# ErikNatanael/knaster

Hardware: AMD Instinct MI355X
Metric: UGen-samples/sec (voices x block_size x UGens / s) (higher is better)
Workload: dtype f32

## Files before the change

knaster_amd/csrc/bank.hip:

```cpp
#include <hip/hip_runtime.h>

#include <algorithm>
#include <atomic>
#include <chrono>
#include <cmath>
#include <cstddef>
#include <cstdio>
#include <cstdlib>
#include <cstring>
#include <functional>
#include <memory>
#include <mutex>
#include <new>
#include <stdexcept>
#include <string>
#include <thread>
#include <vector>

#include "../../include/knaster_hip.h"
#include "jit.hpp"
#include "kernel_form.hpp"
#include "kernel_registry.hpp"

using knh_dev::Event;
// ... 310 lines not shown
    return create_bank(desc, k >= 2 && k <= 64 ? static_cast<uint32_t>(k) : 0u, out_bank);
  });
}

int32_t knh_bank_create_sharded(const knh_bank_desc* desc, uint32_t host_threads, knh_bank** out_bank) {
  return guarded(nullptr, [&]() -> int32_t {
    return create_bank(desc, host_threads, out_bank);
  });
}

void knh_bank_destroy(knh_bank* bank) {
  try {
    if (bank && bank->pipe_stream) {
      (void)hipSetDevice(bank->device);
      (void)hipStreamSynchronize(bank->pipe_stream);
    }
    delete bank;
  } catch (...) {
  }
}

int32_t knh_bank_set_ctor_args(knh_bank* bank, uint32_t stage, uint32_t first_voice, uint32_t count, const double* args, uint32_t n_args) {
  return guarded(bank, [&]() -> int32_t {
    if (!bank) return KNH_ERR_INVALID_ARGUMENT;
    return bank->set_ctor(stage, first_voice, count, args, n_args);
  });
}
int32_t knh_bank_set_buffer(knh_bank* bank, uint32_t stage, const void* samples, size_t n_frames, double buffer_sample_rate) {
  return guarded(bank, [&]() -> int32_t {
    if (!bank) return KNH_ERR_INVALID_ARGUMENT;
// ... 226 lines not shown
int32_t knh_bank_process_blocks_device_add(knh_bank* bank, uint32_t n_blocks, uint64_t frame_clock, void* out_device, void* hip_stream) {
  return guarded(bank, [&]() -> int32_t {
    if (!bank) return KNH_ERR_INVALID_ARGUMENT;
    return bank->process(n_blocks, bank->block_size, 0, frame_clock, nullptr, out_device, nullptr, nullptr, hip_stream, false, true);
  });
}
int32_t knh_bank_process_blocks_begin(knh_bank* bank, uint32_t n_blocks, uint64_t frame_clock) {
  return guarded(bank, [&]() -> int32_t {
    if (!bank) return KNH_ERR_INVALID_ARGUMENT;
    if (!bank->initialised) return bank->fail(KNH_ERR_NOT_INITIALISED, "bank not initialised");
    if (bank->pipe_count == 2) return bank->fail(KNH_ERR_INVALID_ARGUMENT, "two launches are outstanding: fetch one with knh_bank_process_blocks_end first");
    if (n_blocks == 0 || n_blocks > 4096) return bank->fail(KNH_ERR_INVALID_ARGUMENT, "n_blocks must be in 1..4096");
    auto hip = [&](hipError_t e, const char* what) { return e == hipSuccess ? KNH_OK : bank->fail(KNH_ERR_DEVICE, std::string(what) + ": " + hipGetErrorString(e)); };
    int rc = hip(hipSetDevice(bank->device), "hipSetDevice");
    if (rc != KNH_OK) return rc;
    if (!bank->pipe_stream && (rc = hip(hipStreamCreateWithFlags(&bank->pipe_stream, hipStreamNonBlocking), "hipStreamCreate")) != KNH_OK) return rc;
    knh_bank::PipeSlot& p = bank->pipe[(bank->pipe_head + bank->pipe_count) % 2];
    const size_t bytes = static_cast<size_t>(n_blocks) * bank->desc.out_channels * bank->block_size * (bank->desc.sample_type == KNH_F64 ? 8 : 4);
    if (bytes > p.cap) {
      if (p.dev) (void)hipFree(p.dev);
      if (p.host) (void)hipHostFree(p.host);
      p.dev = p.host = nullptr;
      p.cap = 0;
      if ((rc = hip(hipMalloc(&p.dev, bytes), "hipMalloc")) != KNH_OK) return rc;
      if ((rc = hip(hipMemset(p.dev, 0, bytes), "hipMemset")) != KNH_OK) return rc;
      if ((rc = hip(hipHostMalloc(&p.host, bytes), "hipHostMalloc")) != KNH_OK) return rc;
      p.cap = bytes;
    }
    if (!p.done && (rc = hip(hipEventCreateWithFlags(&p.done, hipEventDisableTiming), "hipEventCreate")) != KNH_OK) return rc;
    p.bytes = bytes;
    rc = bank->process(n_blocks, bank->block_size, 0, frame_clock, nullptr, p.dev, nullptr, nullptr, bank->pipe_stream, false);
// ... 132 lines not shown
```

knaster_amd/csrc/kernel_registry.hpp:

```cpp
#pragma once
#include <hip/hip_runtime.h>

#include "voice_chain.hpp"

namespace knh_dev {
enum { INTERP_VAL_MUL = 0, INTERP_VAL_ADD, INTERP_VAL_SUB, INTERP_VAL_DIV, INTERP_VAL_VSUB, INTERP_VAL_VDIV, INTERP_VAL_LAST = INTERP_VAL_VDIV,
       INTERP_MATH_MUL, INTERP_MATH_ADD, INTERP_MATH_SUB, INTERP_MATH_DIV, INTERP_SIN_WT,
       INTERP_MATH1_CEIL, INTERP_MATH1_SQRT, INTERP_MATH1_FLOOR, INTERP_MATH1_TRUNC, INTERP_MATH1_FRACT, INTERP_MATH1_EXP };
struct InterpOp { u32 kind; unsigned short a, b, o, pad; u32 slot; };
static_assert(sizeof(InterpOp) == 16, "one 16-byte LDS read per stage");
struct DevRec {
  u32 voice;
  unsigned short delay;
  unsigned short stage;
  unsigned char param;
  unsigned char kb;
  unsigned short block;
  u32 pad;
  u64 value;
};
static_assert(sizeof(DevRec) == 24, "one 24-byte record per call");
struct DevStage {
  unsigned short kind, dcpb, slot_base, param_base, flags, ar_param;
  short widx;
// ... 30 lines not shown
  u32 seg_max;
  void* delay_ring;
  u32 n_rings;
  u64 ring_base[16];
  u32 ring_stride[16];
};
}

namespace knh {
hipError_t launch_resolve_events(const knh_dev::EventResolveArgs& a, hipStream_t s);
hipError_t launch_restart_voices(const knh_dev::RestartArgs& a, unsigned count, hipStream_t s);

template <typename F>
using VoiceLaunchFn = hipError_t (*)(const knh_dev::VoiceKernelArgs<F>& args, unsigned n_wavefronts, hipStream_t stream);

struct KernelEntry {
  const char* signature;
  int n_slots;
  VoiceLaunchFn<float> f32[2];
  VoiceLaunchFn<double> f64[2];
};
struct PipeEntry {
  const char* signature;
  int n_groups;
  int form;
  int gpw;
  int long_tiles;
  VoiceLaunchFn<float> f32[2];
  VoiceLaunchFn<double> f64[2];
};
// ... 14 lines not shown
hipError_t launch_interp_f64(const knh_dev::VoiceKernelArgs<double>& a, const knh_dev::InterpOp* prog, unsigned n_ops, unsigned n_state_words,
                             unsigned n_sig, unsigned out_sig, double* rows, hipStream_t s);

const KernelEntry* find_kernel(const char* signature);
int kernel_count();
const KernelEntry* kernel_at(int i);

hipError_t launch_res_server_f32(const knh_dev::ResServerArgs<float>& a, hipStream_t s);
hipError_t launch_res_server_f64(const knh_dev::ResServerArgs<double>& a, hipStream_t s);
hipError_t launch_fold_f32(bool tree, const float* rows, unsigned n_rows, unsigned row_len, unsigned frame_begin,
                           unsigned frame_end, float* out, unsigned channels, unsigned out_stride, unsigned n_blocks, bool accumulate,
                           unsigned* zero_flags, hipStream_t s, const knh_dev::HostDone* host = nullptr);
hipError_t launch_fold_f64(bool tree, const double* rows, unsigned n_rows, unsigned row_len, unsigned frame_begin,
                           unsigned frame_end, double* out, unsigned channels, unsigned out_stride, unsigned n_blocks, bool accumulate,
                           unsigned* zero_flags, hipStream_t s, const knh_dev::HostDone* host = nullptr);

hipError_t launch_sum_shards_f32(const float* shards, unsigned n_shards, size_t shard_stride, size_t n, unsigned block_size,
                                 unsigned frame_begin, unsigned frame_end, float* out, bool accumulate, hipStream_t s);
hipError_t launch_sum_shards_f64(const double* shards, unsigned n_shards, size_t shard_stride, size_t n, unsigned block_size,
                                 unsigned frame_begin, unsigned frame_end, double* out, bool accumulate, hipStream_t s);

}
```

knaster_amd/csrc/kernels_fold.hip:

```cpp
#include <cstring>

#include "kernel_registry.hpp"
#include "voice_pipe.hpp"

namespace knh {
using namespace knh_dev;

template <typename F>
static hipError_t launch_fold(bool tree, const F* rows, unsigned n_rows, unsigned row_len, unsigned frame_begin, unsigned frame_end,
                              F* out, unsigned channels, unsigned out_stride, unsigned n_blocks, bool accumulate, unsigned* zero_flags,
                              const HostDone& host, hipStream_t s) {
  if (frame_end <= frame_begin || n_rows == 0 || n_blocks == 0) {
    if (host.words) return hipErrorInvalidValue;
    return zero_flags ? hipMemsetAsync(zero_flags, 0, 2 * sizeof(unsigned), s) : hipSuccess;
  }
  if (tree) {
    unsigned grid = (frame_end - frame_begin + 15u) / 16u;
    hipLaunchKernelGGL((fold_tree_kernel<F>), dim3(grid, n_blocks), dim3(256), 0, s, rows, n_rows, row_len, frame_begin, frame_end,
                       out, channels, out_stride, accumulate ? 1u : 0u, zero_flags, host);
  } else {
    unsigned grid = (frame_end - frame_begin + 63u) / 64u;
    hipLaunchKernelGGL((fold_rows_kernel<F>), dim3(grid, n_blocks), dim3(64), 0, s, rows, n_rows, row_len, frame_begin, frame_end,
                       out, channels, out_stride, accumulate ? 1u : 0u, zero_flags, host);
  }
  return hipGetLastError();
}
hipError_t launch_fold_f32(bool tree, const float* rows, unsigned n_rows, unsigned row_len, unsigned frame_begin,
                           unsigned frame_end, float* out, unsigned channels, unsigned out_stride, unsigned n_blocks, bool accumulate,
                           unsigned* zero_flags, hipStream_t s, const knh_dev::HostDone* host) {
  return launch_fold<float>(tree, rows, n_rows, row_len, frame_begin, frame_end, out, channels, out_stride, n_blocks, accumulate, zero_flags,
                            host ? *host : HostDone{nullptr, nullptr, nullptr, 0u}, s);
}
hipError_t launch_fold_f64(bool tree, const double* rows, unsigned n_rows, unsigned row_len, unsigned frame_begin,
                           unsigned frame_end, double* out, unsigned channels, unsigned out_stride, unsigned n_blocks, bool accumulate,
                           unsigned* zero_flags, hipStream_t s, const knh_dev::HostDone* host) {
  return launch_fold<double>(tree, rows, n_rows, row_len, frame_begin, frame_end, out, channels, out_stride, n_blocks, accumulate, zero_flags,
                             host ? *host : HostDone{nullptr, nullptr, nullptr, 0u}, s);
}


hipError_t launch_res_server_f32(const knh_dev::ResServerArgs<float>& a, hipStream_t s) {
  hipLaunchKernelGGL((res_fold_server<float>), dim3((a.n_rows + 31u) / 32u + 1u), dim3(256), 0, s, a);
  return hipGetLastError();
}
hipError_t launch_res_server_f64(const knh_dev::ResServerArgs<double>& a, hipStream_t s) {
  hipLaunchKernelGGL((res_fold_server<double>), dim3((a.n_rows + 31u) / 32u + 1u), dim3(256), 0, s, a);
  return hipGetLastError();
}

template <typename F>
__global__ void __launch_bounds__(256) sum_shards_kernel(const F* shards, unsigned n_shards, size_t shard_stride, size_t n,
                                                         unsigned block_size, unsigned frame_begin, unsigned frame_end, F* out,
                                                         unsigned accumulate) {
  const size_t i = (size_t)blockIdx.x * 256u + threadIdx.x;
// ... 26 lines not shown
```

knaster_amd/csrc/kernels_pipe.hip:

```cpp
#include <cstring>

#include "kernel_registry.hpp"
#include "voice_pipe.hpp"

namespace knh {
using namespace knh_dev;

template <typename F, bool FMA, int FORM, typename... Gs>
static hipError_t launch_pipe(const VoiceKernelArgs<F>& args, unsigned n_wavefronts, hipStream_t stream) {
  if (n_wavefronts == 0) return hipSuccess;
  constexpr int T = FORM != PIPE_MIXER ? PipeTile<F>::big : PipeTile<F>::value;
  hipLaunchKernelGGL((voice_pipe_kernel<F, FMA, T, FORM, 1, Gs...>), dim3(n_wavefronts), dim3(PipeWaves<T, FORM, Gs...>::value * 64), 0, stream, args);
  return hipGetLastError();
}
template <typename F, bool FMA, typename... Gs>
static hipError_t launch_pipe_pair(const VoiceKernelArgs<F>& args, unsigned n_wavefronts, hipStream_t stream) {
  if (n_wavefronts == 0) return hipSuccess;
  constexpr int T = PipeTile<F>::value;
  hipLaunchKernelGGL((voice_pipe_kernel<F, FMA, T, PIPE_INPLACE, 2, Gs...>), dim3((n_wavefronts + 1u) / 2u),
                     dim3(2 * PipeWaves<T, PIPE_INPLACE, Gs...>::value * 64), 0, stream, args);
  return hipGetLastError();
}
template <typename F, bool FMA, typename... Gs>
static hipError_t launch_pipe_wide_tile(const VoiceKernelArgs<F>& args, unsigned n_wavefronts, hipStream_t stream) {
  if (n_wavefronts == 0) return hipSuccess;
  constexpr int T = PipeTile<F>::big;
  hipLaunchKernelGGL((voice_pipe_kernel<F, FMA, T, PIPE_MIXER, 1, Gs...>), dim3(n_wavefronts), dim3(PipeWaves<T, PIPE_MIXER, Gs...>::value * 64), 0, stream, args);
  return hipGetLastError();
}
#define KNH_PIPE_FAN(sig, n, ...)                                                                                       \
  {sig, n, PIPE_MIXER, 1, 1, {launch_pipe_wide_tile<float, false, __VA_ARGS__>, launch_pipe_wide_tile<float, true, __VA_ARGS__>}, \
   {launch_pipe_wide_tile<double, false, __VA_ARGS__>, launch_pipe_wide_tile<double, true, __VA_ARGS__>}}
#define KNH_PIPE_AS(sig, n, form, ...)                                                               \
  {sig, n, form, 1, form != PIPE_MIXER ? 1 : 0, {launch_pipe<float, false, form, __VA_ARGS__>, launch_pipe<float, true, form, __VA_ARGS__>}, \
   {launch_pipe<double, false, form, __VA_ARGS__>, launch_pipe<double, true, form, __VA_ARGS__>}}
#define KNH_PIPE_PAIR_AS(sig, n, ...)                                                                \
  {sig, n, PIPE_INPLACE, 2, 0, {launch_pipe_pair<float, false, __VA_ARGS__>, launch_pipe_pair<float, true, __VA_ARGS__>}, \
   {launch_pipe_pair<double, false, __VA_ARGS__>, launch_pipe_pair<double, true, __VA_ARGS__>}},
#ifndef KNH_PIPE_PART
#error "KNH_PIPE_PART: 0, 1 or 2 (knaster_amd/build.py)"
#endif
#if KNH_PIPE_PART == 0
// ... 88 lines not shown
```

knaster_amd/csrc/kernels_single.hip:

```cpp
#include <cstring>

#include "kernel_registry.hpp"
#include "voice_pipe.hpp"

namespace knh {
using namespace knh_dev;

template <typename F, bool FMA, typename... S>
static hipError_t launch_voice(const VoiceKernelArgs<F>& args, unsigned n_wavefronts, hipStream_t stream) {
  if (n_wavefronts == 0) return hipSuccess;
  hipLaunchKernelGGL((voice_kernel<F, FMA, 1, S...>), dim3(n_wavefronts), dim3(64), 0, stream, args);
  return hipGetLastError();
}

#define KNH_CHAIN(sig, ...)                                                                  \
  {sig, Chain<float, false, 0, __VA_ARGS__>::kSlots,                                         \
   {launch_voice<float, false, __VA_ARGS__>, launch_voice<float, true, __VA_ARGS__>},        \
   {launch_voice<double, false, __VA_ARGS__>, launch_voice<double, true, __VA_ARGS__>}}

static const KernelEntry kEntries[] = {
    KNH_CHAIN("Wm", SinWt, MulVal),
    KNH_CHAIN("Nm", SinNum, MulVal),
    KNH_CHAIN("WmSA", SinWt, MulVal, Svf, MulAsr),
    KNH_CHAIN("WmaRm", SinWt, MulVal, AddVal, SinWtAr, MulVal),
    KNH_CHAIN("W", SinWt),
    KNH_CHAIN("N", SinNum),
// ... 29 lines not shown
```

knaster_amd/csrc/kernels_wide.hip:

```cpp
#include <cstring>

#include "kernel_registry.hpp"
#include "voice_pipe.hpp"

namespace knh {
using namespace knh_dev;

template <typename F, bool FMA, int WAVES, typename... S>
static hipError_t launch_wide(const VoiceKernelArgs<F>& args, unsigned n_wavefronts, hipStream_t stream) {
  if (n_wavefronts == 0) return hipSuccess;
  hipLaunchKernelGGL((voice_kernel<F, FMA, WAVES, S...>), dim3((n_wavefronts + WAVES - 1) / WAVES), dim3(WAVES * 64), 0, stream, args);
  return hipGetLastError();
}
#define KNH_WIDE(sig, ...)                                                                            \
  {sig,                                                                                               \
   {launch_wide<float, false, 4, __VA_ARGS__>, launch_wide<float, true, 4, __VA_ARGS__>},            \
   {launch_wide<float, false, 8, __VA_ARGS__>, launch_wide<float, true, 8, __VA_ARGS__>},            \
   {launch_wide<double, false, 4, __VA_ARGS__>, launch_wide<double, true, 4, __VA_ARGS__>},          \
   {launch_wide<double, false, 8, __VA_ARGS__>, launch_wide<double, true, 8, __VA_ARGS__>},          \
   {launch_wide<float, false, 16, __VA_ARGS__>, launch_wide<float, true, 16, __VA_ARGS__>},          \
   {launch_wide<double, false, 16, __VA_ARGS__>, launch_wide<double, true, 16, __VA_ARGS__>}}
#define KNH_WIDE_RINGS(sig, ...)                                                                      \
  {sig,                                                                                               \
   {launch_wide<float, false, 4, __VA_ARGS__>, launch_wide<float, true, 4, __VA_ARGS__>},            \
   {launch_wide<float, false, 4, __VA_ARGS__>, launch_wide<float, true, 4, __VA_ARGS__>},            \
   {launch_wide<double, false, 4, __VA_ARGS__>, launch_wide<double, true, 4, __VA_ARGS__>},          \
// ... 24 lines not shown
```

knaster_amd/csrc/voice_bank.hpp:

```cpp
#pragma once

namespace {

template <typename F>
struct Bank final : knh_bank {
  typedef typename knh_dev::WordOf<F>::type W;
  struct ChosenForm {
    knh::FormCandidate is;
    knh::FormFacts facts;
    knh::VoiceLaunchFn<F> fn = nullptr;
    const knh::JitKernel* jit = nullptr;
  } form;
  std::vector<knh_dev::InterpOp> h_prog;
  knh_dev::InterpOp* d_prog = nullptr;
  unsigned interp_sigs = 0, interp_out = 0;
  uint32_t* d_sin_slots = nullptr;
  unsigned frame_vpw = 1, n_sin = 0;
  uint64_t env_ranks = 0;
  std::string signature;
  const char* debug_signature() const override { return signature.c_str(); }
  void set_outputs(bool conn, uint32_t left, uint32_t right, const std::string& sig) override {
    knh_bank::set_outputs(conn, left, right, sig);
    signature = sig;
  }
// ... 143 lines not shown
  std::vector<DelayRings> rings;
  std::vector<int> ring_of_stage;
  std::vector<uint32_t> delay_len;
  uint32_t& ring_len(size_t stage, uint32_t v) { return delay_len[static_cast<size_t>(ring_of_stage[stage]) * nv + v]; }
  uint32_t ring_row(size_t stage, uint32_t v) const {
    const DelayRings& r = rings[static_cast<size_t>(ring_of_stage[stage])];
    return static_cast<uint32_t>((r.base + static_cast<uint64_t>(v) * r.stride) / kRingGranule);
  }
  std::vector<double> env_start;
  std::vector<uint32_t> env_nseg;
  F* d_partials = nullptr;
  F* d_out = nullptr;
  F* d_voices = nullptr;
  uint32_t* d_done = nullptr;
  uint32_t* d_flags = nullptr;
  uint32_t flags_parity = 0;
  uint32_t* flags_last = nullptr;
  hipStream_t flags_stream = nullptr;
  bool flags_stream_set = false;
  uint32_t* h_ev_start2[2] = {nullptr, nullptr};
  Event* h_events2[2] = {nullptr, nullptr};
  size_t h_events_cap2[2] = {0, 0};
  hipEvent_t list_done[2] = {nullptr, nullptr};
  bool list_busy[2] = {false, false};
  unsigned list_parity = 0;
  int list_in_use = -1;
  uint32_t* h_ev_start = nullptr;
  Event* h_events = nullptr;
  F* h_out = nullptr;
  uint32_t* h_done = nullptr;
  uint32_t* d_fold_count = nullptr;
  uint32_t done_epoch = 0;
  ResidentCall<F> resident;
  void resident_stats(uint64_t* calls, uint64_t* launches) override { resident.stats(calls, launches); }
// ... 31 lines not shown
    a.res = knh_dev::Resident{};
    a.n_ranges = 0;
  }
  bool timing = false;
  std::vector<std::pair<hipEvent_t, hipEvent_t>> timing_pool;
  size_t timing_used = 0;
  double timing_ms = 0.0;
  uint64_t timing_launches = 0;

  ~Bank() override {
    if (device >= 0) (void)hipSetDevice(device);
    (void)resident.leave();
    if (own_stream) (void)hipStreamSynchronize(own_stream);
    resolver.quiesce();
    if (flags_stream_set && flags_stream != own_stream) (void)hipStreamSynchronize(flags_stream);
    void* dev_ptrs[] = {d_state, d_sine, d_seg_table, d_delay, d_buffer, d_wavetables, d_partials, d_out, d_voices, d_done, d_flags, d_input, d_prog, d_sin_slots, d_fold_count};
    for (void* p : dev_ptrs)
      if (p) (void)hipFree(p);
    void* host_ptrs[] = {h_ev_start2[0], h_ev_start2[1], h_events2[0], h_events2[1], h_out, h_input, h_done, h_rs_voices, h_rs_words, h_rs_seg};
    for (void* p : host_ptrs)
      if (p) (void)hipHostFree(p);
    for (hipEvent_t e : list_done)
      if (e) (void)hipEventDestroy(e);
    if (in_copied) (void)hipEventDestroy(in_copied);
    if (rs_done) (void)hipEventDestroy(rs_done);
    for (auto& p : timing_pool) {
      (void)hipEventDestroy(p.first);
      (void)hipEventDestroy(p.second);
    }
    if (own_stream) (void)hipStreamDestroy(own_stream);
  }
// ... 651 lines not shown
      KNH_HIP(hipMemcpy(d_prog, h_prog.data(), h_prog.size() * sizeof(knh_dev::InterpOp), hipMemcpyHostToDevice));
      std::vector<uint32_t> sins;
      for (const knh_dev::InterpOp& op : h_prog)
        if (op.kind == knh_dev::INTERP_SIN_WT) sins.push_back(op.slot);
      n_sin = static_cast<unsigned>(sins.size());
      KNH_HIP(hipMalloc(&d_sin_slots, std::max<size_t>(1, sins.size()) * sizeof(uint32_t)));
      if (!sins.empty()) KNH_HIP(hipMemcpy(d_sin_slots, sins.data(), sins.size() * sizeof(uint32_t), hipMemcpyHostToDevice));
    }
    pan = !sig.empty() && (stages.back().kind == KNH_STAGE_PAN2 || connected);
    fold_planes = pan ? 2u : 1u;
    KNH_HIP(hipMalloc(&d_partials, fold_planes * n_waves * bs * sizeof(F)));
    KNH_HIP(hipMalloc(&d_out, desc.out_channels * bs * sizeof(F)));
    KNH_HIP(hipMemset(d_out, 0, desc.out_channels * bs * sizeof(F)));
    KNH_HIP(hipMalloc(&d_done, static_cast<size_t>(nv) * sizeof(uint32_t)));
    KNH_HIP(hipMemset(d_done, 0xFF, static_cast<size_t>(nv) * sizeof(uint32_t)));
    KNH_HIP(hipMalloc(&d_flags, 48 * sizeof(uint32_t)));
    KNH_HIP(hipMemset(d_flags, 0, 48 * sizeof(uint32_t)));
    for (int b = 0; b < 2; ++b) {
      KNH_HIP(hipHostMalloc(&h_ev_start2[b], (static_cast<size_t>(nv) + 2) * sizeof(uint32_t)));
      h_events_cap2[b] = std::max<size_t>(2048, 2 * static_cast<size_t>(nv));
      KNH_HIP(hipHostMalloc(&h_events2[b], h_events_cap2[b] * sizeof(Event)));
      KNH_HIP(hipEventCreateWithFlags(&list_done[b], hipEventDisableTiming));
    }
    KNH_HIP(hipHostMalloc(&h_out, desc.out_channels * bs * sizeof(F) + 2 * sizeof(uint32_t), hipHostMallocMapped | hipHostMallocCoherent));
    KNH_HIP(hipHostMalloc(&h_done, 64, hipHostMallocMapped | hipHostMallocCoherent));
    std::memset(h_done, 0, 64);
    KNH_HIP(hipMalloc(&d_fold_count, sizeof(uint32_t)));
    KNH_HIP(hipMemset(d_fold_count, 0, sizeof(uint32_t)));
    if (desc.mix_mode == KNH_MIX_LEFT_FOLD) KNH_HIP(ensure_voices());
    bool any_wrapped = false;
    for (auto& S : stages) any_wrapped = any_wrapped || S.dcpb > 0;
    if (any_wrapped) next_delay.assign(static_cast<size_t>(n_params_total) * nv, 0);
// ... 34 lines not shown
    {
      typename ResidentCall<F>::Setup rs{};
      rs.bank = this;
      rs.own_stream = own_stream;
      rs.n_rows = (nv + 63u) / 64u;
      rs.fold_planes = fold_planes;
      rs.out_channels = desc.out_channels;
      rs.block_size = static_cast<uint32_t>(bs);
      rs.tile_frames = form.facts.tile_frames;
      rs.can_finish = can_finish;
      rs.ev_start = h_ev_start2;
      rs.events = h_events2;
      rs.launch_voice = [this](const knh_dev::Resident& r) {
        VoiceKernelArgs<F> a;
        fill_launch_args(a, 1, 0, static_cast<uint32_t>(block_size));
        a.flags = d_flags + 32;
        a.res = r;
        return launch_voice(a, (nv + 63) / 64, own_stream);
      };
      resident.setup(rs);
    }
    signature = sig;
    initialised = true;
    return KNH_OK;
  }
  bool can_finish = false;
  bool pan = false;
  F* stage_out = nullptr;
  unsigned fold_planes = 1;
  hipError_t ensure_voices() {
    if (d_voices) return hipSuccess;
// ... 870 lines not shown
    return KNH_OK;
  }

  int process(uint32_t n_blocks, size_t ftp, size_t offset, uint64_t , void* out_host, void* out_device, void* voices_host,
              uint32_t* out_flags, void* stream, bool sync, bool accumulate) override {
    if (accumulate && !out_device) return fail(KNH_ERR_INVALID_ARGUMENT, "accumulation needs a device output buffer");
    if (!initialised) return fail(KNH_ERR_NOT_INITIALISED, "bank not initialised");
    if (offset + ftp > block_size) return fail(KNH_ERR_INVALID_ARGUMENT, "block_start_offset + frames_to_process exceeds block_size");
    if (n_blocks == 0 || n_blocks > 4096) return fail(KNH_ERR_INVALID_ARGUMENT, "n_blocks must be in 1..4096");
    if (n_blocks > 1 && (offset != 0 || ftp != block_size)) return fail(KNH_ERR_INVALID_ARGUMENT, "multi-block launches process whole blocks");
    if (n_blocks > 1 && voices_host) return fail(KNH_ERR_INVALID_ARGUMENT, "per-voice output is only available for single blocks");
    KNH_HIP(hipSetDevice(device));
    hipStream_t s = stream ? static_cast<hipStream_t>(stream) : own_stream;
    if (resolver.take_overflow()) warn("Not enough space for scheduled changes in WrPreciseTiming, change ignored");
    const uint32_t fb = static_cast<uint32_t>(offset), fe = static_cast<uint32_t>(offset + ftp);
    { int rr = flush_restart(s); if (rr != KNH_OK) return rr; }
    mid_block = fe < block_size;
    for (uint32_t b = 0; b < n_blocks; ++b) {
      frame_base = b * static_cast<uint32_t>(block_size);
      if (b > 0 && b < future.size()) {
        for (const Call& c : future[b]) {
          if (c.is_delay) set_delay(c.voice, c.stage, c.param, c.delay);
          else param_apply(c.voice, c.stage, c.param, c.kind, c.f, c.i);
        }
      }
      if (b < qfuture.size()) resolve_qrecs(qfuture[b], fb, fe);
      resolve_queues(fb, fe);
    }
    frame_base = 0;
    if (!qfuture.empty()) {
// ... 36 lines not shown
          if (rc != KNH_OK) return rc;
        }
      }
      resident.sat_out();
      rc = resident.leave();
      if (rc != KNH_OK) return rc;
      ResidentCall<F>::make_room(device, this);
    }
    const bool want_voices = voices_host != nullptr || (desc.mix_mode == KNH_MIX_LEFT_FOLD) || stage_out != nullptr;
    if (desc.mix_mode == KNH_MIX_LEFT_FOLD && n_blocks > 1)
      return fail(KNH_ERR_INVALID_ARGUMENT, "KNH_MIX_LEFT_FOLD processes one block per call");
    if (stage_out && n_blocks > 1) return fail(KNH_ERR_INTERNAL, "a bank that feeds a following stage renders one block per launch");
    if (want_voices && !stage_out) KNH_HIP(ensure_voices());
    const bool rows_per_voice = form.facts.rows_per_voice;
    const unsigned n_waves = rows_per_voice ? nv : (nv + 63) / 64;
    if (n_blocks > partials_blocks) {
      KNH_HIP(hipStreamSynchronize(s));
      KNH_HIP(hipFree(d_partials));
      d_partials = nullptr;
      KNH_HIP(hipMalloc(&d_partials, static_cast<size_t>(n_blocks) * fold_planes * n_waves * block_size * sizeof(F)));
      partials_blocks = n_blocks;
    }
    if (!out_device && n_blocks > out_blocks) {
      KNH_HIP(hipStreamSynchronize(s));
      KNH_HIP(hipFree(d_out));
      d_out = nullptr;
      KNH_HIP(hipMalloc(&d_out, static_cast<size_t>(n_blocks) * desc.out_channels * block_size * sizeof(F)));
      KNH_HIP(hipMemsetAsync(d_out, 0, static_cast<size_t>(n_blocks) * desc.out_channels * block_size * sizeof(F), s));
      if (h_out) KNH_HIP(hipHostFree(h_out));
      h_out = nullptr;
      KNH_HIP(hipHostMalloc(&h_out, static_cast<size_t>(n_blocks) * desc.out_channels * block_size * sizeof(F) + 2 * sizeof(uint32_t),
                            hipHostMallocMapped | hipHostMallocCoherent));
      out_blocks = n_blocks;
    }

    if (flags_stream_set && flags_stream != s) KNH_HIP(hipStreamSynchronize(flags_stream));
    flags_stream = s;
    flags_stream_set = true;
    uint32_t* const flags_now = d_flags + 16 * flags_parity;
    uint32_t* const flags_next = d_flags + 16 * (flags_parity ^ 1u);
    flags_parity ^= 1u;
    flags_last = flags_now;
    VoiceKernelArgs<F> a;
    fill_launch_args(a, n_blocks, fb, fe);
    if (uses_input) {
      if (in_blocks_set != n_blocks) return fail(KNH_ERR_INVALID_ARGUMENT, "a bank with KNH_STAGE_INPUT stages needs knh_bank_set_input for exactly the blocks of this call");
      if (in_device) {
        a.input = in_device;
      } else {
        if (in_host_pending) {
          KNH_HIP(hipMemcpyAsync(d_input, h_input, static_cast<size_t>(n_blocks) * desc.in_channels * block_size * sizeof(F), hipMemcpyHostToDevice, s));
          if (!in_copied) KNH_HIP(hipEventCreateWithFlags(&in_copied, hipEventDisableTiming));
          KNH_HIP(hipEventRecord(in_copied, s));
          in_copy_pending = true;
        }
        in_host_pending = false;
        a.input = d_input;
      }
      in_blocks_set = 0;
    }
    a.ev_start = have_events && !launch_n_ranges ? h_ev_start : nullptr;
    a.events = h_events;
    if (launch_n_ranges) {
      a.n_ranges = launch_n_ranges;
      std::copy(launch_range_recs, launch_range_recs + 2 * launch_n_ranges, a.ranges);
      ev_range_launches += 1;
    } else if (have_events) {
      ev_list_launches += 1;
      ev_list_bytes += static_cast<uint64_t>(h_ev_start[nv]) * sizeof(Event) + (static_cast<uint64_t>(nv) + 1u) * sizeof(uint32_t);
    }
    if (resolver.pending()) {
      DevEventResolver::Lists lists{};
      int r2 = resolver.resolve(s, n_blocks, fb, fe, have_events ? h_ev_start : nullptr, h_events, have_events ? h_ev_start[nv] : 0u, &lists);
      if (r2 != KNH_OK) return r2;
      a.ev_start = lists.ev_start;
      a.events = lists.events;
      if (!have_events) ev_list_launches += 1;
    }
    a.voices_out = want_voices ? (stage_out ? stage_out : d_voices) : nullptr;
    a.flags = flags_now;
    std::pair<hipEvent_t, hipEvent_t>* tp = nullptr;
    if (timing) {
      if (timing_used == timing_pool.size()) {
        if (timing_pool.size() >= 8192) {
          int r = timing_collect();
          if (r != KNH_OK) return r;
        } else {
          hipEvent_t e0, e1;
          KNH_HIP(hipEventCreate(&e0));
          KNH_HIP(hipEventCreate(&e1));
          timing_pool.emplace_back(e0, e1);
        }
      }
      tp = &timing_pool[timing_used++];
      KNH_HIP(hipEventRecord(tp->first, s));
    }
    KNH_HIP(rows_per_voice ? launch_frames(a, s) : launch_voice(a, n_waves, s));
    if (tp) KNH_HIP(hipEventRecord(tp->second, s));
    if (stage_out && rows_per_voice)
      KNH_HIP(hipMemcpyAsync(stage_out, d_partials, static_cast<size_t>(nv) * block_size * sizeof(F), hipMemcpyDeviceToDevice, s));
    { int r2 = resolver.kernel_enqueued(s); if (r2 != KNH_OK) return r2; }
    if (have_events && list_in_use >= 0) {
      KNH_HIP(hipEventRecord(list_done[list_in_use], s));
      list_busy[list_in_use] = true;
      list_in_use = -1;
    }

    const bool hand_over = sync && out_host && !out_device && !voices_host && fe > fb;
    F* dst = out_device ? static_cast<F*>(out_device) : (hand_over ? h_out : d_out);
    knh_dev::HostDone hd{nullptr, nullptr, nullptr, 0u};
    if (hand_over) {
      done_epoch += 1;
      if (done_epoch == 0) done_epoch = 1;
      hd = knh_dev::HostDone{h_done, d_fold_count, flags_now, done_epoch};
    }
    const unsigned fold_channels = pan ? 1u : desc.out_channels;
    if (desc.mix_mode == KNH_MIX_LEFT_FOLD)
      KNH_HIP(launch_fold(false, rows_per_voice ? d_partials : d_voices, nv, static_cast<unsigned>(block_size), fb, fe, dst, fold_channels, static_cast<unsigned>(block_size), fold_planes, accumulate, flags_next, s, hand_over ? &hd : nullptr));
    else
      KNH_HIP(launch_fold(true, d_partials, n_waves, static_cast<unsigned>(block_size), fb, fe, dst, fold_channels, static_cast<unsigned>(block_size), n_blocks * fold_planes, accumulate, flags_next, s, hand_over ? &hd : nullptr));

    if (!sync) return KNH_OK;
    const size_t blk_elems = desc.out_channels * block_size;
    const size_t out_bytes = static_cast<size_t>(n_blocks) * blk_elems * sizeof(F);
    uint32_t* h_flags = reinterpret_cast<uint32_t*>(reinterpret_cast<char*>(h_out) + static_cast<size_t>(out_blocks) * blk_elems * sizeof(F));
    if (hand_over) {
      volatile uint32_t* ep = h_done;
      for (uint64_t spin = 1;; ++spin) {
        if (__atomic_load_n(ep, __ATOMIC_ACQUIRE) == done_epoch) break;
        if ((spin & 0x3FFFu) == 0) {
          const hipError_t q = hipStreamQuery(s);
          if (q == hipSuccess) {
            if (__atomic_load_n(ep, __ATOMIC_ACQUIRE) == done_epoch) break;
            KNH_HIP(hipStreamSynchronize(s));
// ... 38 lines not shown
    else return knh::launch_interp_f64(a, d_prog, n_ops, n_words, interp_sigs, interp_out, rows, s);
  }
  hipError_t launch_voice(const VoiceKernelArgs<F>& a, unsigned n_waves, hipStream_t s) {
    return form.jit ? knh::jit_launch(form.jit, &a, sizeof(a), n_waves, s) : form.fn(a, n_waves, s);
  }
  knh::VoiceLaunchFn<F> launch_fn(const knh::VoiceLaunchFn<float> (&f32)[2], const knh::VoiceLaunchFn<double> (&f64)[2]) const {
    if constexpr (sizeof(F) == 4) return f32[desc.allow_fma ? 1 : 0];
    else return f64[desc.allow_fma ? 1 : 0];
  }
  static hipError_t launch_fold(bool tree, const float* rows, unsigned n, unsigned len, unsigned fb, unsigned fe, float* out, unsigned ch, unsigned os, unsigned nb, bool acc, uint32_t* zf, hipStream_t s, const knh_dev::HostDone* hd) {
    return knh::launch_fold_f32(tree, rows, n, len, fb, fe, out, ch, os, nb, acc, zf, s, hd);
  }
  static hipError_t launch_fold(bool tree, const double* rows, unsigned n, unsigned len, unsigned fb, unsigned fe, double* out, unsigned ch, unsigned os, unsigned nb, bool acc, uint32_t* zf, hipStream_t s, const knh_dev::HostDone* hd) {
    return knh::launch_fold_f64(tree, rows, n, len, fb, fe, out, ch, os, nb, acc, zf, s, hd);
  }

  int read_done_frames(uint32_t* out) override {
    if (!initialised) return fail(KNH_ERR_NOT_INITIALISED, "bank not initialised");
    if (!out) return fail(KNH_ERR_INVALID_ARGUMENT, "null output");
    { int rl = resident.leave(); if (rl != KNH_OK) return rl; }
    KNH_HIP(hipSetDevice(device));
    { int rr = flush_restart(own_stream); if (rr != KNH_OK) return rr; }
    KNH_HIP(hipStreamSynchronize(own_stream));
    KNH_HIP(hipMemcpy(out, d_done, static_cast<size_t>(nv) * sizeof(uint32_t), hipMemcpyDeviceToHost));
    return KNH_OK;
  }
  int debug_read(uint32_t* out16) override {
    if (!initialised) return fail(KNH_ERR_NOT_INITIALISED, "bank not initialised");
    { int rl = resident.leave(); if (rl != KNH_OK) return rl; }
    KNH_HIP(hipSetDevice(device));
    KNH_HIP(hipDeviceSynchronize());
    KNH_HIP(hipMemcpy(out16, flags_last ? flags_last : d_flags, 16 * sizeof(uint32_t), hipMemcpyDeviceToHost));
    out16[2] = form.is.kind;
    out16[3] = !form.facts.rows_per_voice ? 0u
             : form.jit ? frame_vpw
             : knh::interp_voices_per_workgroup(nv, static_cast<unsigned>(h_prog.size()), static_cast<unsigned>(n_slots), interp_sigs, static_cast<unsigned>(block_size), sizeof(F) == 8);
    return KNH_OK;
  }
  int synchronize() override {
    if (!initialised) return fail(KNH_ERR_NOT_INITIALISED, "bank not initialised");
    { int rl = resident.leave(); if (rl != KNH_OK) return rl; }
    KNH_HIP(hipSetDevice(device));
    KNH_HIP(hipDeviceSynchronize());
    return KNH_OK;
  }
  int timing_collect() {
    KNH_HIP(hipDeviceSynchronize());
    for (size_t k = 0; k < timing_used; ++k) {
      float ms = 0.f;
      KNH_HIP(hipEventElapsedTime(&ms, timing_pool[k].first, timing_pool[k].second));
      timing_ms += ms;
// ... 29 lines not shown
```

knaster_amd/csrc/voice_chain.hpp:

```cpp
#pragma once
#include "voice_stages.hpp"

namespace knh_dev {

template <typename F, bool FMA, int BASE, typename... S> struct Chain;
template <typename F, bool FMA, int BASE>
struct Chain<F, FMA, BASE> {
  static constexpr int kSlots = BASE;
  static constexpr bool kUsesSine = false;
  static constexpr bool kPan = false;
  static constexpr bool kStereo = false;
  static constexpr u64 kParamBits = 0ull, kNopOkBits = 0ull;
  static constexpr bool kBinds = false;
  static constexpr bool kBlockWork = false;
  static constexpr bool kUsesRing = false;
  static constexpr int kRingStages = 0;
  template <int T> __device__ __forceinline__ void tick_tile_sw(const Chain&, u32, u64, F (&)[T], const Ctx&, u32) {}
  __device__ __forceinline__ void pan_gains(F&, F&) const {}
  template <typename W> __device__ __forceinline__ void load(const W*, long) {}
  template <typename W> __device__ __forceinline__ void store(W*, long) const {}
  __device__ __forceinline__ F tick(F x, const Ctx&, u32) { return x; }
  template <int T> __device__ __forceinline__ void tick_tile(F (&)[T], const Ctx&, u32) {}
  static constexpr bool kRunFixed = false;
  struct RunPrep {};
// ... 1196 lines not shown
      }
    }
    __syncthreads();
  }
  if (g == 0 && in_range) {
    F total = stack[depth - 1][f];
    for (u32 d = depth - 1; d > 0; --d) total = stack[d - 1][f] + total;
    for (u32 c = 0; c < channels; ++c) {
      F* o = out + (long)c * out_stride + n;
      *o = accumulate ? *o + total : total;
    }
  }
  fold_signal_host(host);
}

}
```

Measured before the change: 3543 billion.

## Overlap voice kernels with wave-level tree fold on separate prioritized streams

Voice rendering now runs on a high-priority stream and the partial-row fold on a low-priority stream. Double-buffered partials and a three-way flags rotation let one call's fold overlap the next call's voice kernel. A new single-wave tree-fold kernel reduces up to 256 rows in registers without shared-memory synchronisation. Launch events are carried through a thread-local hook into hipExtLaunchKernelGGL. This adds event bookkeeping and extra memory, and it can deadlock or mis-order work if a launcher ignores the hook.

```diff
diff --git a/knaster_amd/csrc/bank.hip b/knaster_amd/csrc/bank.hip
--- a/knaster_amd/csrc/bank.hip
+++ b/knaster_amd/csrc/bank.hip
@@ -348,6 +348,7 @@
     if (bank && bank->pipe_stream) {
       (void)hipSetDevice(bank->device);
       (void)hipStreamSynchronize(bank->pipe_stream);
+      host_pipe_streams().remove(bank->pipe_stream);
     }
     delete bank;
   } catch (...) {
@@ -604,7 +605,10 @@
     auto hip = [&](hipError_t e, const char* what) { return e == hipSuccess ? KNH_OK : bank->fail(KNH_ERR_DEVICE, std::string(what) + ": " + hipGetErrorString(e)); };
     int rc = hip(hipSetDevice(bank->device), "hipSetDevice");
     if (rc != KNH_OK) return rc;
-    if (!bank->pipe_stream && (rc = hip(hipStreamCreateWithFlags(&bank->pipe_stream, hipStreamNonBlocking), "hipStreamCreate")) != KNH_OK) return rc;
+    if (!bank->pipe_stream) {
+      if ((rc = hip(hipStreamCreateWithFlags(&bank->pipe_stream, hipStreamNonBlocking), "hipStreamCreate")) != KNH_OK) return rc;
+      host_pipe_streams().add(bank->pipe_stream);
+    }
     knh_bank::PipeSlot& p = bank->pipe[(bank->pipe_head + bank->pipe_count) % 2];
     const size_t bytes = static_cast<size_t>(n_blocks) * bank->desc.out_channels * bank->block_size * (bank->desc.sample_type == KNH_F64 ? 8 : 4);
     if (bytes > p.cap) {
diff --git a/knaster_amd/csrc/kernel_registry.hpp b/knaster_amd/csrc/kernel_registry.hpp
--- a/knaster_amd/csrc/kernel_registry.hpp
+++ b/knaster_amd/csrc/kernel_registry.hpp
@@ -1,5 +1,6 @@
 #pragma once
 #include <hip/hip_runtime.h>
+#include <hip/hip_ext.h>
 
 #include "voice_chain.hpp"
 
@@ -68,6 +69,19 @@
 template <typename F>
 using VoiceLaunchFn = hipError_t (*)(const knh_dev::VoiceKernelArgs<F>& args, unsigned n_wavefronts, hipStream_t stream);
 
+struct LaunchEvents { hipEvent_t start = nullptr, stop = nullptr; };
+LaunchEvents& launch_events();
+template <typename K, typename A>
+inline void launch_voice_kernel(K kernel, dim3 grid, dim3 block, hipStream_t stream, const A& args) {
+  LaunchEvents& ev = launch_events();
+  if (ev.start || ev.stop) {
+    hipExtLaunchKernelGGL(kernel, grid, block, 0, stream, ev.start, ev.stop, 0, args);
+    ev = LaunchEvents{};
+  } else {
+    hipLaunchKernelGGL(kernel, grid, block, 0, stream, args);
+  }
+}
+
 struct KernelEntry {
   const char* signature;
   int n_slots;
@@ -112,6 +126,10 @@
 hipError_t launch_fold_f64(bool tree, const double* rows, unsigned n_rows, unsigned row_len, unsigned frame_begin,
                            unsigned frame_end, double* out, unsigned channels, unsigned out_stride, unsigned n_blocks, bool accumulate,
                            unsigned* zero_flags, hipStream_t s, const knh_dev::HostDone* host = nullptr);
+hipError_t launch_fold_wave_f32(const float* rows, unsigned n_rows, unsigned row_len, unsigned frame_begin, unsigned frame_end, float* out,
+                                unsigned channels, unsigned out_stride, unsigned n_blocks, bool accumulate, unsigned* zero_flags, hipStream_t s);
+hipError_t launch_fold_wave_f64(const double* rows, unsigned n_rows, unsigned row_len, unsigned frame_begin, unsigned frame_end, double* out,
+                                unsigned channels, unsigned out_stride, unsigned n_blocks, bool accumulate, unsigned* zero_flags, hipStream_t s);
 
 hipError_t launch_sum_shards_f32(const float* shards, unsigned n_shards, size_t shard_stride, size_t n, unsigned block_size,
                                  unsigned frame_begin, unsigned frame_end, float* out, bool accumulate, hipStream_t s);
diff --git a/knaster_amd/csrc/kernels_fold.hip b/knaster_amd/csrc/kernels_fold.hip
--- a/knaster_amd/csrc/kernels_fold.hip
+++ b/knaster_amd/csrc/kernels_fold.hip
@@ -5,6 +5,11 @@
 
 namespace knh {
 using namespace knh_dev;
+
+LaunchEvents& launch_events() {
+  static thread_local LaunchEvents ev;
+  return ev;
+}
 
 template <typename F>
 static hipError_t launch_fold(bool tree, const F* rows, unsigned n_rows, unsigned row_len, unsigned frame_begin, unsigned frame_end,
@@ -38,6 +43,23 @@
                              host ? *host : HostDone{nullptr, nullptr, nullptr, 0u}, s);
 }
 
+template <typename F>
+static hipError_t launch_fold_wave(const F* rows, unsigned n_rows, unsigned row_len, unsigned frame_begin, unsigned frame_end, F* out,
+                                   unsigned channels, unsigned out_stride, unsigned n_blocks, bool accumulate, unsigned* zero_flags, hipStream_t s) {
+  if (frame_end <= frame_begin || n_rows == 0 || n_rows > 256 || n_blocks == 0) return hipErrorInvalidValue;
+  const unsigned grid = (frame_end - frame_begin + 63u) / 64u;
+  hipLaunchKernelGGL((fold_tree_wave_kernel<F>), dim3(grid, n_blocks), dim3(64), 0, s, rows, n_rows, row_len, frame_begin, frame_end, out,
+                     channels, out_stride, accumulate ? 1u : 0u, zero_flags);
+  return hipGetLastError();
+}
+hipError_t launch_fold_wave_f32(const float* rows, unsigned n_rows, unsigned row_len, unsigned frame_begin, unsigned frame_end, float* out,
+                                unsigned channels, unsigned out_stride, unsigned n_blocks, bool accumulate, unsigned* zero_flags, hipStream_t s) {
+  return launch_fold_wave<float>(rows, n_rows, row_len, frame_begin, frame_end, out, channels, out_stride, n_blocks, accumulate, zero_flags, s);
+}
+hipError_t launch_fold_wave_f64(const double* rows, unsigned n_rows, unsigned row_len, unsigned frame_begin, unsigned frame_end, double* out,
+                                unsigned channels, unsigned out_stride, unsigned n_blocks, bool accumulate, unsigned* zero_flags, hipStream_t s) {
+  return launch_fold_wave<double>(rows, n_rows, row_len, frame_begin, frame_end, out, channels, out_stride, n_blocks, accumulate, zero_flags, s);
+}
 
 hipError_t launch_res_server_f32(const knh_dev::ResServerArgs<float>& a, hipStream_t s) {
   hipLaunchKernelGGL((res_fold_server<float>), dim3((a.n_rows + 31u) / 32u + 1u), dim3(256), 0, s, a);
diff --git a/knaster_amd/csrc/kernels_pipe.hip b/knaster_amd/csrc/kernels_pipe.hip
--- a/knaster_amd/csrc/kernels_pipe.hip
+++ b/knaster_amd/csrc/kernels_pipe.hip
@@ -10,22 +10,22 @@
 static hipError_t launch_pipe(const VoiceKernelArgs<F>& args, unsigned n_wavefronts, hipStream_t stream) {
   if (n_wavefronts == 0) return hipSuccess;
   constexpr int T = FORM != PIPE_MIXER ? PipeTile<F>::big : PipeTile<F>::value;
-  hipLaunchKernelGGL((voice_pipe_kernel<F, FMA, T, FORM, 1, Gs...>), dim3(n_wavefronts), dim3(PipeWaves<T, FORM, Gs...>::value * 64), 0, stream, args);
+  launch_voice_kernel(voice_pipe_kernel<F, FMA, T, FORM, 1, Gs...>, dim3(n_wavefronts), dim3(PipeWaves<T, FORM, Gs...>::value * 64), stream, args);
   return hipGetLastError();
 }
 template <typename F, bool FMA, typename... Gs>
 static hipError_t launch_pipe_pair(const VoiceKernelArgs<F>& args, unsigned n_wavefronts, hipStream_t stream) {
   if (n_wavefronts == 0) return hipSuccess;
   constexpr int T = PipeTile<F>::value;
-  hipLaunchKernelGGL((voice_pipe_kernel<F, FMA, T, PIPE_INPLACE, 2, Gs...>), dim3((n_wavefronts + 1u) / 2u),
-                     dim3(2 * PipeWaves<T, PIPE_INPLACE, Gs...>::value * 64), 0, stream, args);
+  launch_voice_kernel(voice_pipe_kernel<F, FMA, T, PIPE_INPLACE, 2, Gs...>, dim3((n_wavefronts + 1u) / 2u),
+                      dim3(2 * PipeWaves<T, PIPE_INPLACE, Gs...>::value * 64), stream, args);
   return hipGetLastError();
 }
 template <typename F, bool FMA, typename... Gs>
 static hipError_t launch_pipe_wide_tile(const VoiceKernelArgs<F>& args, unsigned n_wavefronts, hipStream_t stream) {
   if (n_wavefronts == 0) return hipSuccess;
   constexpr int T = PipeTile<F>::big;
-  hipLaunchKernelGGL((voice_pipe_kernel<F, FMA, T, PIPE_MIXER, 1, Gs...>), dim3(n_wavefronts), dim3(PipeWaves<T, PIPE_MIXER, Gs...>::value * 64), 0, stream, args);
+  launch_voice_kernel(voice_pipe_kernel<F, FMA, T, PIPE_MIXER, 1, Gs...>, dim3(n_wavefronts), dim3(PipeWaves<T, PIPE_MIXER, Gs...>::value * 64), stream, args);
   return hipGetLastError();
 }
 #define KNH_PIPE_FAN(sig, n, ...)                                                                                       \
diff --git a/knaster_amd/csrc/kernels_single.hip b/knaster_amd/csrc/kernels_single.hip
--- a/knaster_amd/csrc/kernels_single.hip
+++ b/knaster_amd/csrc/kernels_single.hip
@@ -9,7 +9,7 @@
 template <typename F, bool FMA, typename... S>
 static hipError_t launch_voice(const VoiceKernelArgs<F>& args, unsigned n_wavefronts, hipStream_t stream) {
   if (n_wavefronts == 0) return hipSuccess;
-  hipLaunchKernelGGL((voice_kernel<F, FMA, 1, S...>), dim3(n_wavefronts), dim3(64), 0, stream, args);
+  launch_voice_kernel(voice_kernel<F, FMA, 1, S...>, dim3(n_wavefronts), dim3(64), stream, args);
   return hipGetLastError();
 }
 
diff --git a/knaster_amd/csrc/kernels_wide.hip b/knaster_amd/csrc/kernels_wide.hip
--- a/knaster_amd/csrc/kernels_wide.hip
+++ b/knaster_amd/csrc/kernels_wide.hip
@@ -9,7 +9,7 @@
 template <typename F, bool FMA, int WAVES, typename... S>
 static hipError_t launch_wide(const VoiceKernelArgs<F>& args, unsigned n_wavefronts, hipStream_t stream) {
   if (n_wavefronts == 0) return hipSuccess;
-  hipLaunchKernelGGL((voice_kernel<F, FMA, WAVES, S...>), dim3((n_wavefronts + WAVES - 1) / WAVES), dim3(WAVES * 64), 0, stream, args);
+  launch_voice_kernel(voice_kernel<F, FMA, WAVES, S...>, dim3((n_wavefronts + WAVES - 1) / WAVES), dim3(WAVES * 64), stream, args);
   return hipGetLastError();
 }
 #define KNH_WIDE(sig, ...)                                                                            \
diff --git a/knaster_amd/csrc/voice_bank.hpp b/knaster_amd/csrc/voice_bank.hpp
--- a/knaster_amd/csrc/voice_bank.hpp
+++ b/knaster_amd/csrc/voice_bank.hpp
@@ -1,6 +1,18 @@
 #pragma once
 
 namespace {
+
+struct HostPipeStreams {
+  std::mutex m;
+  std::vector<hipStream_t> streams;
+  void add(hipStream_t s) { std::lock_guard<std::mutex> l(m); streams.push_back(s); }
+  void remove(hipStream_t s) { std::lock_guard<std::mutex> l(m); streams.erase(std::remove(streams.begin(), streams.end(), s), streams.end()); }
+  bool has(hipStream_t s) { std::lock_guard<std::mutex> l(m); return std::find(streams.begin(), streams.end(), s) != streams.end(); }
+};
+inline HostPipeStreams& host_pipe_streams() {
+  static HostPipeStreams h;
+  return h;
+}
 
 template <typename F>
 struct Bank final : knh_bank {
@@ -181,10 +193,36 @@
   F* d_voices = nullptr;
   uint32_t* d_done = nullptr;
   uint32_t* d_flags = nullptr;
-  uint32_t flags_parity = 0;
+  uint32_t flags_turn = 0;
   uint32_t* flags_last = nullptr;
   hipStream_t flags_stream = nullptr;
   bool flags_stream_set = false;
+  bool fold_overlap = [] { const char* e = std::getenv("KNH_FOLD_OVERLAP"); return !(e && e[0] == '0'); }();
+  bool fold_wave_always = [] { const char* e = std::getenv("KNH_FOLD_WAVE"); return e && e[0] == '1'; }();
+  hipStream_t voice_stream = nullptr, fold_stream = nullptr;
+  hipEvent_t caller_at = nullptr;
+  hipEvent_t voice_done[2] = {nullptr, nullptr};
+  hipEvent_t fold_done[2] = {nullptr, nullptr};
+  bool fold_busy[2] = {false, false};
+  F* d_partials2 = nullptr;
+  uint32_t overlap_turn = 0;
+  bool last_overlapped = false;
+  uint64_t overlapped_launches = 0, wave_folds = 0;
+  int ensure_overlap_streams(unsigned n_waves) {
+    if (!voice_stream || !fold_stream) {
+      int least = 0, greatest = 0;
+      KNH_HIP(hipDeviceGetStreamPriorityRange(&least, &greatest));
+      if (!voice_stream) KNH_HIP(hipStreamCreateWithPriority(&voice_stream, hipStreamNonBlocking, greatest));
+      if (!fold_stream) KNH_HIP(hipStreamCreateWithPriority(&fold_stream, hipStreamNonBlocking, least));
+    }
+    if (!caller_at) KNH_HIP(hipEventCreateWithFlags(&caller_at, hipEventDisableTiming));
+    for (int k = 0; k < 2; ++k) {
+      if (!voice_done[k]) KNH_HIP(hipEventCreateWithFlags(&voice_done[k], hipEventDisableTiming));
+      if (!fold_done[k]) KNH_HIP(hipEventCreateWithFlags(&fold_done[k], hipEventDisableTiming));
+    }
+    if (!d_partials2) KNH_HIP(hipMalloc(&d_partials2, static_cast<size_t>(partials_blocks) * fold_planes * n_waves * block_size * sizeof(F)));
+    return KNH_OK;
+  }
   uint32_t* h_ev_start2[2] = {nullptr, nullptr};
   Event* h_events2[2] = {nullptr, nullptr};
   size_t h_events_cap2[2] = {0, 0};
@@ -246,7 +284,14 @@
     if (own_stream) (void)hipStreamSynchronize(own_stream);
     resolver.quiesce();
     if (flags_stream_set && flags_stream != own_stream) (void)hipStreamSynchronize(flags_stream);
-    void* dev_ptrs[] = {d_state, d_sine, d_seg_table, d_delay, d_buffer, d_wavetables, d_partials, d_out, d_voices, d_done, d_flags, d_input, d_prog, d_sin_slots, d_fold_count};
+    for (hipStream_t st : {voice_stream, fold_stream})
+      if (st) { (void)hipStreamSynchronize(st); (void)hipStreamDestroy(st); }
+    if (caller_at) (void)hipEventDestroy(caller_at);
+    for (int k = 0; k < 2; ++k) {
+      if (voice_done[k]) (void)hipEventDestroy(voice_done[k]);
+      if (fold_done[k]) (void)hipEventDestroy(fold_done[k]);
+    }
+    void* dev_ptrs[] = {d_state, d_sine, d_seg_table, d_delay, d_buffer, d_wavetables, d_partials, d_partials2, d_out, d_voices, d_done, d_flags, d_input, d_prog, d_sin_slots, d_fold_count};
     for (void* p : dev_ptrs)
       if (p) (void)hipFree(p);
     void* host_ptrs[] = {h_ev_start2[0], h_ev_start2[1], h_events2[0], h_events2[1], h_out, h_input, h_done, h_rs_voices, h_rs_words, h_rs_seg};
@@ -928,8 +973,8 @@
     KNH_HIP(hipMemset(d_out, 0, desc.out_channels * bs * sizeof(F)));
     KNH_HIP(hipMalloc(&d_done, static_cast<size_t>(nv) * sizeof(uint32_t)));
     KNH_HIP(hipMemset(d_done, 0xFF, static_cast<size_t>(nv) * sizeof(uint32_t)));
-    KNH_HIP(hipMalloc(&d_flags, 48 * sizeof(uint32_t)));
-    KNH_HIP(hipMemset(d_flags, 0, 48 * sizeof(uint32_t)));
+    KNH_HIP(hipMalloc(&d_flags, 64 * sizeof(uint32_t)));
+    KNH_HIP(hipMemset(d_flags, 0, 64 * sizeof(uint32_t)));
     for (int b = 0; b < 2; ++b) {
       KNH_HIP(hipHostMalloc(&h_ev_start2[b], (static_cast<size_t>(nv) + 2) * sizeof(uint32_t)));
       h_events_cap2[b] = std::max<size_t>(2048, 2 * static_cast<size_t>(nv));
@@ -994,7 +1039,7 @@
       rs.launch_voice = [this](const knh_dev::Resident& r) {
         VoiceKernelArgs<F> a;
         fill_launch_args(a, 1, 0, static_cast<uint32_t>(block_size));
-        a.flags = d_flags + 32;
+        a.flags = d_flags + 48;
         a.res = r;
         return launch_voice(a, (nv + 63) / 64, own_stream);
       };
@@ -1895,6 +1940,7 @@
     hipStream_t s = stream ? static_cast<hipStream_t>(stream) : own_stream;
     if (resolver.take_overflow()) warn("Not enough space for scheduled changes in WrPreciseTiming, change ignored");
     const uint32_t fb = static_cast<uint32_t>(offset), fe = static_cast<uint32_t>(offset + ftp);
+    const bool restart_flushed = !rs_voices.empty();
     { int rr = flush_restart(s); if (rr != KNH_OK) return rr; }
     mid_block = fe < block_size;
     for (uint32_t b = 0; b < n_blocks; ++b) {
@@ -1961,13 +2007,24 @@
     if (want_voices && !stage_out) KNH_HIP(ensure_voices());
     const bool rows_per_voice = form.facts.rows_per_voice;
     const unsigned n_waves = rows_per_voice ? nv : (nv + 63) / 64;
+    const bool overlap_now = fold_overlap && !sync && out_device && !voices_host && !stage_out && desc.mix_mode == KNH_MIX_TREE &&
+                             form.facts.walks_ranges && !rows_per_voice && n_waves <= 256u && fe > fb && !host_pipe_streams().has(s);
     if (n_blocks > partials_blocks) {
       KNH_HIP(hipStreamSynchronize(s));
+      if (voice_stream) KNH_HIP(hipStreamSynchronize(voice_stream));
+      if (fold_stream) KNH_HIP(hipStreamSynchronize(fold_stream));
+      const size_t bytes = static_cast<size_t>(n_blocks) * fold_planes * n_waves * block_size * sizeof(F);
       KNH_HIP(hipFree(d_partials));
       d_partials = nullptr;
-      KNH_HIP(hipMalloc(&d_partials, static_cast<size_t>(n_blocks) * fold_planes * n_waves * block_size * sizeof(F)));
+      KNH_HIP(hipMalloc(&d_partials, bytes));
+      if (d_partials2) {
+        KNH_HIP(hipFree(d_partials2));
+        d_partials2 = nullptr;
+        KNH_HIP(hipMalloc(&d_partials2, bytes));
+      }
       partials_blocks = n_blocks;
     }
+    if (overlap_now) { int r2 = ensure_overlap_streams(n_waves); if (r2 != KNH_OK) return r2; }
     if (!out_device && n_blocks > out_blocks) {
       KNH_HIP(hipStreamSynchronize(s));
       KNH_HIP(hipFree(d_out));
@@ -1984,9 +2041,9 @@
     if (flags_stream_set && flags_stream != s) KNH_HIP(hipStreamSynchronize(flags_stream));
     flags_stream = s;
     flags_stream_set = true;
-    uint32_t* const flags_now = d_flags + 16 * flags_parity;
-    uint32_t* const flags_next = d_flags + 16 * (flags_parity ^ 1u);
-    flags_parity ^= 1u;
+    uint32_t* const flags_now = d_flags + 16 * flags_turn;
+    uint32_t* const flags_next = d_flags + 16 * ((flags_turn + 2u) % 3u);
+    flags_turn = (flags_turn + 1u) % 3u;
     flags_last = flags_now;
     VoiceKernelArgs<F> a;
     fill_launch_args(a, n_blocks, fb, fe);
@@ -2006,6 +2063,16 @@
       }
       in_blocks_set = 0;
     }
+    hipStream_t vs = s;
+    const uint32_t row_set = overlap_now ? overlap_turn : 0u;
+    if (overlap_now) {
+      overlap_turn ^= 1u;
+      vs = voice_stream;
+      a.partials = row_set ? d_partials2 : d_partials;
+      KNH_HIP(hipEventRecord(caller_at, s));
+      if (!last_overlapped || uses_input || restart_flushed) KNH_HIP(hipStreamWaitEvent(vs, caller_at, 0));
+      if (fold_busy[row_set]) KNH_HIP(hipEventSynchronize(fold_done[row_set]));
+    }
     a.ev_start = have_events && !launch_n_ranges ? h_ev_start : nullptr;
     a.events = h_events;
     if (launch_n_ranges) {
@@ -2018,7 +2085,7 @@
     }
     if (resolver.pending()) {
       DevEventResolver::Lists lists{};
-      int r2 = resolver.resolve(s, n_blocks, fb, fe, have_events ? h_ev_start : nullptr, h_events, have_events ? h_ev_start[nv] : 0u, &lists);
+      int r2 = resolver.resolve(vs, n_blocks, fb, fe, have_events ? h_ev_start : nullptr, h_events, have_events ? h_ev_start[nv] : 0u, &lists);
       if (r2 != KNH_OK) return r2;
       a.ev_start = lists.ev_start;
       a.events = lists.events;
@@ -2040,15 +2107,24 @@
         }
       }
       tp = &timing_pool[timing_used++];
-      KNH_HIP(hipEventRecord(tp->first, s));
-    }
-    KNH_HIP(rows_per_voice ? launch_frames(a, s) : launch_voice(a, n_waves, s));
-    if (tp) KNH_HIP(hipEventRecord(tp->second, s));
+    }
+    const bool carried = overlap_now && !form.jit;
+    if (tp && !carried) KNH_HIP(hipEventRecord(tp->first, vs));
+    if (carried) knh::launch_events() = tp ? knh::LaunchEvents{tp->first, tp->second} : knh::LaunchEvents{nullptr, voice_done[row_set]};
+    const hipError_t launched = rows_per_voice ? launch_frames(a, vs) : launch_voice(a, n_waves, vs);
+    const bool events_left = knh::launch_events().start || knh::launch_events().stop;
+    knh::launch_events() = knh::LaunchEvents{};
+    KNH_HIP(launched);
+    if (carried && events_left) {
+      (void)hipStreamSynchronize(vs);
+      return fail(KNH_ERR_INTERNAL, "the launcher of this kernel form did not take the launch's events (knh::launch_voice_kernel)");
+    }
+    if (tp && !carried) KNH_HIP(hipEventRecord(tp->second, vs));
     if (stage_out && rows_per_voice)
       KNH_HIP(hipMemcpyAsync(stage_out, d_partials, static_cast<size_t>(nv) * block_size * sizeof(F), hipMemcpyDeviceToDevice, s));
-    { int r2 = resolver.kernel_enqueued(s); if (r2 != KNH_OK) return r2; }
+    { int r2 = resolver.kernel_enqueued(vs); if (r2 != KNH_OK) return r2; }
     if (have_events && list_in_use >= 0) {
-      KNH_HIP(hipEventRecord(list_done[list_in_use], s));
+      KNH_HIP(hipEventRecord(list_done[list_in_use], vs));
       list_busy[list_in_use] = true;
       list_in_use = -1;
     }
@@ -2062,9 +2138,26 @@
       hd = knh_dev::HostDone{h_done, d_fold_count, flags_now, done_epoch};
     }
     const unsigned fold_channels = pan ? 1u : desc.out_channels;
+    if (overlap_now) {
+      if (!carried) KNH_HIP(hipEventRecord(voice_done[row_set], vs));
+      KNH_HIP(hipStreamWaitEvent(fold_stream, carried && tp ? tp->second : voice_done[row_set], 0));
+      KNH_HIP(hipStreamWaitEvent(fold_stream, caller_at, 0));
+      KNH_HIP(launch_fold_wave(a.partials, n_waves, static_cast<unsigned>(block_size), fb, fe, dst, fold_channels, static_cast<unsigned>(block_size), n_blocks * fold_planes, accumulate, flags_next, fold_stream));
+      KNH_HIP(hipEventRecord(fold_done[row_set], fold_stream));
+      fold_busy[row_set] = true;
+      KNH_HIP(hipStreamWaitEvent(s, fold_done[row_set], 0));
+      last_overlapped = true;
+      overlapped_launches += 1;
+      wave_folds += 1;
+      return KNH_OK;
+    }
+    last_overlapped = false;
     if (desc.mix_mode == KNH_MIX_LEFT_FOLD)
       KNH_HIP(launch_fold(false, rows_per_voice ? d_partials : d_voices, nv, static_cast<unsigned>(block_size), fb, fe, dst, fold_channels, static_cast<unsigned>(block_size), fold_planes, accumulate, flags_next, s, hand_over ? &hd : nullptr));
-    else
+    else if (fold_wave_always && !hand_over && n_waves <= 256u && fe > fb) {
+      KNH_HIP(launch_fold_wave(d_partials, n_waves, static_cast<unsigned>(block_size), fb, fe, dst, fold_channels, static_cast<unsigned>(block_size), n_blocks * fold_planes, accumulate, flags_next, s));
+      wave_folds += 1;
+    } else
       KNH_HIP(launch_fold(true, d_partials, n_waves, static_cast<unsigned>(block_size), fb, fe, dst, fold_channels, static_cast<unsigned>(block_size), n_blocks * fold_planes, accumulate, flags_next, s, hand_over ? &hd : nullptr));
 
     if (!sync) return KNH_OK;
@@ -2133,6 +2226,12 @@
   static hipError_t launch_fold(bool tree, const double* rows, unsigned n, unsigned len, unsigned fb, unsigned fe, double* out, unsigned ch, unsigned os, unsigned nb, bool acc, uint32_t* zf, hipStream_t s, const knh_dev::HostDone* hd) {
     return knh::launch_fold_f64(tree, rows, n, len, fb, fe, out, ch, os, nb, acc, zf, s, hd);
   }
+  static hipError_t launch_fold_wave(const float* rows, unsigned n, unsigned len, unsigned fb, unsigned fe, float* out, unsigned ch, unsigned os, unsigned nb, bool acc, uint32_t* zf, hipStream_t s) {
+    return knh::launch_fold_wave_f32(rows, n, len, fb, fe, out, ch, os, nb, acc, zf, s);
+  }
+  static hipError_t launch_fold_wave(const double* rows, unsigned n, unsigned len, unsigned fb, unsigned fe, double* out, unsigned ch, unsigned os, unsigned nb, bool acc, uint32_t* zf, hipStream_t s) {
+    return knh::launch_fold_wave_f64(rows, n, len, fb, fe, out, ch, os, nb, acc, zf, s);
+  }
 
   int read_done_frames(uint32_t* out) override {
     if (!initialised) return fail(KNH_ERR_NOT_INITIALISED, "bank not initialised");
@@ -2154,6 +2253,10 @@
     out16[3] = !form.facts.rows_per_voice ? 0u
              : form.jit ? frame_vpw
              : knh::interp_voices_per_workgroup(nv, static_cast<unsigned>(h_prog.size()), static_cast<unsigned>(n_slots), interp_sigs, static_cast<unsigned>(block_size), sizeof(F) == 8);
+#ifndef KNH_DAG_STAMPS
+    out16[9] = static_cast<uint32_t>(overlapped_launches);
+    out16[10] = static_cast<uint32_t>(wave_folds);
+#endif
     return KNH_OK;
   }
   int synchronize() override {
diff --git a/knaster_amd/csrc/voice_chain.hpp b/knaster_amd/csrc/voice_chain.hpp
--- a/knaster_amd/csrc/voice_chain.hpp
+++ b/knaster_amd/csrc/voice_chain.hpp
@@ -1234,4 +1234,35 @@
   fold_signal_host(host);
 }
 
-}
+template <typename F>
+__global__ void __launch_bounds__(64) fold_tree_wave_kernel(const F* rows, u32 n_rows, u32 row_len, u32 frame_begin,
+                                                             u32 frame_end, F* out, u32 channels, u32 out_stride, u32 accumulate, u32* zero_flags) {
+  if (zero_flags && blockIdx.x == 0 && blockIdx.y == 0 && threadIdx.x == 0) { zero_flags[0] = 0u; zero_flags[1] = 0u; }
+  const u32 n = frame_begin + blockIdx.x * 64u + threadIdx.x;
+  if (n >= frame_end) return;
+  rows += (long)blockIdx.y * n_rows * row_len;
+  out += (long)blockIdx.y * channels * out_stride;
+  const u32 chunks = (n_rows + 15u) / 16u;
+  F c[16];
+#pragma unroll
+  for (int g = 0; g < 16; ++g) {
+    F acc = (F)0;
+    if ((u32)g < chunks) {
+      const u32 r0 = (u32)g * 16u;
+      const u32 cnt = n_rows - r0 < 16u ? n_rows - r0 : 16u;
+      const F* q = rows + (long)r0 * row_len + n;
+      F v[16];
+#pragma unroll
+      for (int k = 0; k < 16; ++k) v[k] = (u32)k < cnt ? q[(long)k * row_len] : (F)0;
+      acc = cnt == 16u ? tree_reduce<F, 16, true>(v, 1u, 16u) : tree_reduce<F, 16, false>(v, 1u, cnt);
+    }
+    c[g] = acc;
+  }
+  const F total = chunks == 16u ? tree_reduce<F, 16, true>(c, 1u, 16u) : tree_reduce<F, 16, false>(c, 1u, chunks);
+  for (u32 ch = 0; ch < channels; ++ch) {
+    F* o = out + (long)ch * out_stride + n;
+    *o = accumulate ? *o + total : total;
+  }
+}
+
+}
```

Result: faster. 3602 billion, median of 6 (+1.7%).
